# famoreno/stereo-vo

Measured on AMD Instinct MI355X. Metric: stereo pairs/sec @1280×960, higher is better.
Workload: dtype u8/f64

## Files before the change

### stereo_vo_amd/csrc/k_detect.hip

```cpp
#include <algorithm>
#include "svo_device.h"
#include "svo_kernels.h"
#include "../../include/svo_orb_tables.h"

__constant__ int c_umax[16];
__device__ __attribute__((aligned(16))) float4 g_brief_patf[SVO_BRIEF_NPAIRS];
__device__ __attribute__((aligned(16))) uint4 g_blur_gh[3 * 64], g_blur_gv[3 * 64];
#define SVO_DISC_E 256
__device__ uint32_t g_disc_m[SVO_DISC_E], g_disc_x[SVO_DISC_E];
#define DP_REACH SVO_BRIEF_REACH
#define DP_BW (2 * DP_REACH + 1)
#define DP_RW (DP_BW + 6)
#define DP_X0 (DP_REACH + 5)

hipError_t svo_upload_tables()
{
    hipError_t e = hipMemcpyToSymbol(HIP_SYMBOL(c_umax), svo_umax, sizeof(svo_umax));
    if (e != hipSuccess) return e;
    {
        static float4 pf[SVO_BRIEF_NPAIRS];
        for (int i = 0; i < SVO_BRIEF_NPAIRS; i++) pf[i] = make_float4((float)svo_brief_pat[i][0], (float)svo_brief_pat[i][2], (float)svo_brief_pat[i][1], (float)svo_brief_pat[i][3]);
        e = hipMemcpyToSymbol(HIP_SYMBOL(g_brief_patf), pf, sizeof(pf));
        if (e != hipSuccess) return e;
    }
// ... 322 lines not shown
{
    fast_reset(sm.score, sm.s_count, sm.s_nout);
    fast_stage<false>(sm.tile, src, pitch, gw, gh, x0, y0);
    asm volatile("s_waitcnt vmcnt(0)" ::: "memory");
    __syncthreads();
    fast_compute(c, sm.tile, sm.score, sm.list, sm.s_count, sm.s_nout, img, level, gw, gh, x0, y0, th_fast);
}

__device__ __forceinline__ void fast_compute(const DevCtx& c, uint8_t* tile, uint8_t* score, unsigned short* list, unsigned& s_count, unsigned& s_nout,
                                             int img, int level, int gw, int gh, int x0, int y0, int th_fast)
{
    uint32_t* out_keys = (uint32_t*)tile;
    const int tid = threadIdx.x;
    if (c.debug_mode == DBG_FAST_STOP_STAGED) return;
    const uint32_t th = (uint32_t)th_fast;
    const u16x2 t2h = { (unsigned short)(th << 8), (unsigned short)(th << 8) };
    const int gq = tid & (FT_NG - 1), rb = tid >> 4;
    const int e_base = rb * (FT_ROWS * FT_SP) + 4 * gq;
    uint32_t pe[FT_ROWS], po[FT_ROWS];
    {
        const uint32_t* col = (const uint32_t*)tile + rb * (FT_ROWS * (FT_LW / 4)) + gq;
        uint32_t cc[FT_ROWS + 6];
#pragma unroll
        for (int i = 0; i < FT_ROWS + 6; i++) cc[i] = col[i * (FT_LW / 4) + 1];
#pragma unroll
        for (int g = 0; g < FT_ROWS; g++) {
            const uint32_t Cp = col[(g + 3) * (FT_LW / 4)], C = cc[g + 3], Cn = col[(g + 3) * (FT_LW / 4) + 2], N = cc[g], S = cc[g + 6];
            const uint32_t Eo = __builtin_amdgcn_alignbyte(Cn, C, 3), Wo = __builtin_amdgcn_alignbyte(C, Cp, 1);
            const uint32_t Ee = __builtin_amdgcn_alignbyte(Cn, C, 2);
            pe[g] = quick_half(C << 8, N << 8, Ee, S << 8, Cp, t2h);
            po[g] = quick_half(C, N, Eo, S, Wo, t2h);
        }
    }
    auto entry_of = [&](int b) -> int { return e_base + ((b & 7) << 6) + (b >> 3); };
    uint32_t m_left = 0;
    {
        const uint32_t one2 = 0x00010001u;
        uint32_t me = 0, mo = 0;
#pragma unroll
        for (int g = FT_ROWS - 1; g >= 0; g--) {
            uint32_t fe, fo;
            asm("v_pk_min_u16 %0, %1, %2" : "=v"(fe) : "v"(pe[g]), "s"(one2));
            asm("v_pk_min_u16 %0, %1, %2" : "=v"(fo) : "v"(po[g]), "s"(one2));
            if (g == FT_ROWS - 1) { me = fe; mo = fo; }
            else {
                asm("v_lshl_or_b32 %0, %1, 1, %2" : "=v"(me) : "v"(me), "v"(fe));
                asm("v_lshl_or_b32 %0, %1, 1, %2" : "=v"(mo) : "v"(mo), "v"(fo));
            }
        }
        uint32_t m = me | (mo << 8);
        const int cnt = __popc(m), inc = wave_inclusive_scan(cnt);
        const int total = __builtin_amdgcn_readlane(inc, 63);
        if (total) {
            unsigned wbase = 0;
            if ((tid & 63) == 0) wbase = atomicAdd(&s_count, (unsigned)total);
            unsigned idx = (unsigned)__builtin_amdgcn_readfirstlane((int)wbase) + (unsigned)(inc - cnt);
            while (m && idx < FT_LIST_CAP) {
                const int b = __builtin_ctz(m); m &= m - 1;
                list[idx++] = (unsigned short)entry_of(b);
            }
            m_left = m;
        }
    }
    __syncthreads();
    const int ns_all = (int)s_count, ns = min(ns_all, FT_LIST_CAP);
    const bool overflow = ns_all > FT_LIST_CAP;
    if (c.debug_mode == DBG_FAST_STOP_COMPACTED) return;
    auto win_off = [&](int e) -> int { return (e >> 6) * FT_LW + (e & 63) + (3 * FT_LW + 4); };
    for (int i = tid; i < ns; i += FT_NT) {
        const int e = list[i];
        score[e] = (uint8_t)fast_score_lds(tile, win_off(e), th_fast);
    }
    if (__builtin_expect(overflow, 0)) {
        for (uint32_t m = m_left; m; m &= m - 1) {
            const int e = entry_of(__builtin_ctz(m));
            score[e] = (uint8_t)fast_score_lds(tile, win_off(e), th_fast);
        }
    }
    __syncthreads();
    if (c.debug_mode == DBG_FAST_STOP_SCORED) return;
    auto nms_round = [&](bool has, int e) {
        bool keep = false; uint32_t key = 0;
        if (has) {
            const int r = e >> 6, q = e & 63;
            const int nb = e - FT_SP - 1; int nbm = nb; asm volatile("" : "+v"(nbm));
            const int v = score[nbm + FT_SP + 1];
            const int n0 = score[nb], n1 = score[nbm + 1], n2 = score[nb + 2], n3 = score[nb + FT_SP], n4 = score[nb + FT_SP + 2];
            const int n5 = score[nb + 2 * FT_SP], n6 = score[nbm + 2 * FT_SP + 1], n7 = score[nb + 2 * FT_SP + 2];
            const int mx = max(max(max(n0, n1), max(n2, n3)), max(max(n4, n5), max(n6, n7)));
            const int x = x0 - 1 + q, y = y0 - 1 + r;
            keep = (v > mx) & (r >= 1) & (r <= FT_H) & (q >= 1) & (q <= FT_W) & (x < gw - SVO_EDGE) & (y < gh - SVO_EDGE);
            key = ((uint32_t)v << 24) | (0xFFFFFFu - (uint32_t)(y * gw + x));
        }
        const unsigned long long m = __ballot(keep);
        if (m) {
            unsigned b2 = 0;
            const int leader = __ffsll((long long)m) - 1;
            if ((tid & 63) == leader) b2 = atomicAdd(&s_nout, (unsigned)__popcll(m));
            b2 = __shfl(b2, leader, 64);
            if (keep) out_keys[b2 + __popcll(m & ((1ull << (tid & 63)) - 1ull))] = key;
        }
    };
    for (int base = 0; base < ns; base += FT_NT) {
        const int i = base + tid;
        nms_round(i < ns, i < ns ? (int)list[i] : 0);
    }
    if (__builtin_expect(overflow, 0)) {
        uint32_t m = m_left;
        while (__ballot(m != 0)) {
            const bool has = m != 0;
            const int e = has ? entry_of(__builtin_ctz(m)) : 0;
            m &= m - 1;
            nms_round(has, e);
        }
    }
    __syncthreads();
    if (tid < 64) {
        const unsigned nout = s_nout;
        if (nout != 0 && c.debug_mode != DBG_FAST_NO_PUBLISH) {
            const LevelGeom& g = c.lv[level];
            unsigned gbase = 0;
            if (tid == 0) gbase = atomicAdd(&c.cand_cnt[(img * SVO_MAX_LEVELS + level) * SVO_CNT_STRIDE], nout);
            gbase = __shfl(gbase, 0, 64);
            uint32_t* dst = c.cand_keys + (long long)img * c.cand_total + g.cand_off;
            for (unsigned i = tid; i < nout; i += 64) {
                if (gbase + i < (unsigned)g.cand_cap) dst[gbase + i] = out_keys[i];
                else raise_detect_status(c, img >> 1, SVO_ST_CAND_OVERFLOW);
            }
        }
    }
}

__global__ void __launch_bounds__(FT_NT) __attribute__((amdgpu_waves_per_eu(8, 8))) k_fast(DevCtx c)
{
    SVO_TL_SCOPE(c, TL_FAST, 0);
    __shared__ FastSmem sm;
    const uint32_t slot = blockIdx.x >> 3;
    const uint32_t work = c.debug_mode == DBG_LINEAR_TILES ? blockIdx.x : (((slot / FT_CHUNK) * 8 + (blockIdx.x & 7)) * FT_CHUNK + slot % FT_CHUNK);
    const int img = (int)fastdiv(work, c.div_tiles), tile_id = (int)work - img * c.n_tiles;
    if (img >= c.n_img || lane_idle(c, img >> 1)) return;
    const uint4 e = c.fast_tiles[tile_id];
    const uint4 tha = ((const uint4*)(c.fast_th_used + img * SVO_MAX_LEVELS))[0], thb = ((const uint4*)(c.fast_th_used + img * SVO_MAX_LEVELS))[1];
    const uint8_t* base0 = c.img0[img];
    const int level = (int)(e.z & 0xFFu);
    const uint32_t thv[8] = { tha.x, tha.y, tha.z, tha.w, thb.x, thb.y, thb.z, thb.w };
    uint32_t th = thv[0];
#pragma unroll
    for (int l = 1; l < SVO_MAX_LEVELS; l++) th = level == l ? thv[l] : th;
    const uint8_t* src = level == 0 ? base0 : c.pyr + (long long)img * c.pyr_bytes + e.w;
    const int pitch = level == 0 ? c.img0_pitch : (int)(e.z >> 8);
    fast_tile(c, sm, img, level, src, pitch, (int)(e.y & 0xFFFFu), (int)(e.y >> 16), (int)(e.x & 0xFFFFu), (int)(e.x >> 16), (int)th);
}

__global__ void __launch_bounds__(FT_NT) k_fast_redo(DevCtx c)
{
    SVO_TL_SCOPE(c, TL_FAST, 1);
    __shared__ FastSmem sm;
    const unsigned n = *c.redo_n;
    if (n == 0) return;
    int first = (int)blockIdx.x;
    for (unsigned e = 0; e < n; e++) {
        const uint32_t il = c.redo_list[e];
        const int img = (int)(il / SVO_MAX_LEVELS), level = (int)(il % SVO_MAX_LEVELS);
        const int nt = c.lv[level].tiles_x * c.lv[level].tiles_y;
        int t = first;
        int pitch; const uint8_t* src = level_ptr(c, img, level, pitch);
        const int tx = c.lv[level].tiles_x, gw = c.lv[level].w, gh = c.lv[level].h;
        for (; t < nt; t += (int)gridDim.x) {
            const int by = t / tx, bx = t - by * tx;
            fast_tile(c, sm, img, level, src, pitch, gw, gh, SVO_EDGE + bx * FT_W, SVO_EDGE + by * FT_H, c.fast_th);
            __syncthreads();
        }
        first = t - nt;
    }
}


__device__ __forceinline__ float harris_at(const uint8_t* img, int pitch, int x, int y)
{
    int a = 0, b = 0, cc = 0;
    for (int dy = -3; dy <= 3; dy++) {
        const uint8_t* pm = img + (long long)(y + dy - 1) * pitch + x, *p0 = pm + pitch, *pp = p0 + pitch;
#pragma unroll
        for (int dx = -3; dx <= 3; dx++) {
            const int Ix = ((int)p0[dx + 1] - (int)p0[dx - 1]) * 2 + ((int)pm[dx + 1] - (int)pm[dx - 1]) + ((int)pp[dx + 1] - (int)pp[dx - 1]);
            const int Iy = ((int)pp[dx] - (int)pm[dx]) * 2 + ((int)pp[dx - 1] - (int)pm[dx - 1]) + ((int)pp[dx + 1] - (int)pm[dx + 1]);
            a += Ix * Ix; b += Iy * Iy; cc += Ix * Iy;
        }
    }
    const float s = 1.0f / (4.0f * 7.0f * 255.0f);
    const float s4 = s * s * s * s;
    const float fa = (float)a, fb = (float)b, fc = (float)cc;
    const float tr = fa + fb;
    return (fa * fb - fc * fc - 0.04f * tr * tr) * s4;
}

__device__ __forceinline__ float harris_at_dw(const uint8_t* img, int pitch, int x, int y)
{
    const int xa = (x - 4) & ~3, o = (x - 4) & 3;
    int px[9][9];
#pragma unroll
    for (int r = 0; r < 9; r++) {
        const uint3 pw = *(const uint3*)(img + (long long)(y - 4 + r) * pitch + xa);
        const uint32_t w0 = pw.x, w1 = pw.y, w2 = pw.z;
        const uint32_t A = __builtin_amdgcn_alignbyte(w1, w0, o), B = __builtin_amdgcn_alignbyte(w2, w1, o), C = w2 >> (8 * o);
#pragma unroll
        for (int k = 0; k < 4; k++) { px[r][k] = (A >> (8 * k)) & 0xFF; px[r][4 + k] = (B >> (8 * k)) & 0xFF; }
        px[r][8] = C & 0xFF;
    }
    int a = 0, b = 0, cc = 0;
#pragma unroll
    for (int r = 1; r < 8; r++) {
#pragma unroll
        for (int q = 1; q < 8; q++) {
            const int Ix = (px[r][q + 1] - px[r][q - 1]) * 2 + (px[r - 1][q + 1] - px[r - 1][q - 1]) + (px[r + 1][q + 1] - px[r + 1][q - 1]);
            const int Iy = (px[r + 1][q] - px[r - 1][q]) * 2 + (px[r + 1][q - 1] - px[r - 1][q - 1]) + (px[r + 1][q + 1] - px[r - 1][q + 1]);
            a += __mul24(Ix, Ix); b += __mul24(Iy, Iy); cc += __mul24(Ix, Iy);
        }
    }
    const float s = 1.0f / (4.0f * 7.0f * 255.0f);
    const float s4 = s * s * s * s;
    const float fa = (float)a, fb = (float)b, fc = (float)cc;
    const float tr = fa + fb;
    return (fa * fb - fc * fc - 0.04f * tr * tr) * s4;
}

template <int SEL_MAX>
__device__ __forceinline__ int select_block(const DevCtx& c, int redo_pass, int img, int level, unsigned long long* keys, uint32_t* sel, unsigned* hist, int* scan_s, unsigned* sv)
{
    constexpr int SEL_TIE_MAX = 2 * SEL_MAX;
    unsigned& s_prefix = sv[0]; unsigned& s_need = sv[1]; unsigned& s_sel = sv[2]; unsigned& s_tie = sv[3]; unsigned& s_ntie = sv[4];
    const LevelGeom& g = c.lv[level];
    const int tid = threadIdx.x;
    const int il = img * SVO_MAX_LEVELS + level;
    if (redo_pass && !c.redo_flag[il]) return 0;
    unsigned nc = c.cand_cnt[il * SVO_CNT_STRIDE];
    if (nc > (unsigned)g.cand_cap) nc = g.cand_cap;
    const unsigned K = min(nc, (unsigned)(2 * g.quota));
    const uint32_t th_used = c.fast_th_used[il], th_base = (uint32_t)c.fast_th;
    if (!redo_pass && g.quota > 0 && th_used > th_base && nc < (unsigned)(2 * g.quota)) {
        if (tid == 0) {
            c.redo_flag[il] = 1; c.redo_list[atomicAdd(c.redo_n, 1u)] = (uint32_t)il;
            atomicAdd(c.redo_n + 1, 1u);
            c.cand_cnt[il * SVO_CNT_STRIDE] = 0; c.fast_th_used[il] = th_base; c.fast_th_dyn[il] = 0;
        }
        return 0;
    }
    if (K == 0 || g.quota <= 0) { if (tid == 0) { c.lvl_n[il] = 0; c.sel_n[il] = 0; c.fast_th_dyn[il] = 0; } return 0; }
    const uint32_t* ck = c.cand_keys + (long long)img * c.cand_total + g.cand_off;
    uint32_t* tie = (uint32_t*)keys;
    for (int i = tid; i < 256; i += blockDim.x) hist[i] = 0;
    if (tid == 0) { s_sel = 0; s_tie = 0; }
    __syncthreads();
    for (unsigned base = tid; base < nc; base += 8 * 512) {
        uint32_t k[8];
#pragma unroll
        for (int u = 0; u < 8; u++) { const unsigned i = base + u * 512; k[u] = i < nc ? ck[i] : 0u; }
#pragma unroll
        for (int u = 0; u < 8; u++) if (base + u * 512 < nc) atomicAdd(&hist[k[u] >> 24], 1u);
    }
    __syncthreads();
    if (c.debug_mode == DBG_SELECT_STOP_HIST) return 0;
    unsigned prefix = 0, mask = 0, need = K;
    {
        const int mine = tid < 256 ? (int)hist[255 - tid] : 0;
        int tot;
        const int before = block_exclusive_scan(mine, scan_s, &tot);
        if (tid < 256 && (unsigned)before < need && need <= (unsigned)(before + mine)) { s_prefix = (unsigned)(255 - tid) << 24; s_need = need - (unsigned)before; s_ntie = (unsigned)mine; }
        const unsigned M = 3u * (unsigned)g.quota + 32u;
        if (tid < 256 && (unsigned)before < M && M <= (unsigned)(before + mine)) c.fast_th_dyn[il] = (uint32_t)(255 - tid) > th_base ? (uint32_t)(255 - tid) : 0u;
        if (tid == 0 && (unsigned)tot < M) {
            const unsigned dens = max(hist[min(th_used, 255u)], 1u), lower = (M - (unsigned)tot) / dens + 1u;
            c.fast_th_dyn[il] = th_used > th_base + lower ? th_used - lower : 0u;
        }
        __syncthreads();
        prefix = s_prefix; need = s_need; mask = 0xFF000000u;
    }
    const unsigned n_tie = s_ntie;
    uint32_t cutoff;
    const unsigned K_ties = (K - need) + n_tie;
    if (K_ties <= (unsigned)SEL_MAX) {
        cutoff = prefix;
        for (unsigned base = tid; base < nc; base += 8 * 512) {
            uint32_t k[8];
#pragma unroll
            for (int u = 0; u < 8; u++) { const unsigned i = base + u * 512; k[u] = i < nc ? ck[i] : 0u; }
#pragma unroll
            for (int u = 0; u < 8; u++) if (base + u * 512 < nc && k[u] >= cutoff) sel[atomicAdd(&s_sel, 1u)] = k[u];
        }
        __syncthreads();
        return (int)K_ties;
    }
    if (tid == 0) raise_detect_status(c, img >> 1, SVO_ST_CAND_OVERFLOW);
    if (n_tie <= SEL_TIE_MAX) {
        for (unsigned base = tid; base < nc; base += 8 * 512) {
            uint32_t k[8];
#pragma unroll
            for (int u = 0; u < 8; u++) { const unsigned i = base + u * 512; k[u] = i < nc ? ck[i] : 0u; }
#pragma unroll
            for (int u = 0; u < 8; u++) {
                if (base + u * 512 >= nc) continue;
                if ((k[u] & 0xFF000000u) > prefix) sel[atomicAdd(&s_sel, 1u)] = k[u];
                else if ((k[u] & 0xFF000000u) == prefix) tie[atomicAdd(&s_tie, 1u)] = k[u];
            }
        }
        __syncthreads();
        for (int shift = 16; shift >= 0; shift -= 8) {
            for (int i = tid; i < 256; i += blockDim.x) hist[i] = 0;
            __syncthreads();
            for (unsigned i = tid; i < n_tie; i += blockDim.x) { const uint32_t k = tie[i]; if ((k & mask) == prefix) atomicAdd(&hist[(k >> shift) & 255u], 1u); }
            __syncthreads();
            const int mine = tid < 256 ? (int)hist[255 - tid] : 0;
            int tot;
            const int before = block_exclusive_scan(mine, scan_s, &tot);
            if (tid < 256 && (unsigned)before < need && need <= (unsigned)(before + mine)) { s_prefix = prefix | ((unsigned)(255 - tid) << shift); s_need = need - (unsigned)before; }
            __syncthreads();
            prefix = s_prefix; need = s_need; mask |= 255u << shift;
            __syncthreads();
        }
        cutoff = prefix;
        for (unsigned i = tid; i < n_tie; i += blockDim.x) { const uint32_t k = tie[i]; if (k >= cutoff) sel[atomicAdd(&s_sel, 1u)] = k; }
        __syncthreads();
    } else {
        for (int shift = 16; shift >= 0; shift -= 8) {
            for (int i = tid; i < 256; i += blockDim.x) hist[i] = 0;
            __syncthreads();
            for (unsigned i = tid; i < nc; i += blockDim.x) { const uint32_t k = ck[i]; if ((k & mask) == prefix) atomicAdd(&hist[(k >> shift) & 255u], 1u); }
            __syncthreads();
            const int mine = tid < 256 ? (int)hist[255 - tid] : 0;
            int tot;
            const int before = block_exclusive_scan(mine, scan_s, &tot);
            if (tid < 256 && (unsigned)before < need && need <= (unsigned)(before + mine)) { s_prefix = prefix | ((unsigned)(255 - tid) << shift); s_need = need - (unsigned)before; }
            __syncthreads();
            prefix = s_prefix; need = s_need; mask |= 255u << shift;
            __syncthreads();
        }
        cutoff = prefix;
        for (unsigned i = tid; i < nc; i += blockDim.x) { const uint32_t k = ck[i]; if (k >= cutoff) { const unsigned sl = atomicAdd(&s_sel, 1u); if (sl < SEL_MAX) sel[sl] = k; } }
        __syncthreads();
    }
    return (int)K;
}

template <int SEL_MAX>
__global__ void __launch_bounds__(512) k_select(DevCtx c, int redo_pass)
{
    SVO_TL_SCOPE(c, TL_SELECT, redo_pass);
    __shared__ unsigned long long keys[SEL_MAX];
    __shared__ uint32_t sel[SEL_MAX];
    __shared__ unsigned hist[256];
    __shared__ int scan_s[32];
    __shared__ unsigned sv[5];
    const int level = blockIdx.y, img = blockIdx.x, tid = threadIdx.x;
    if (lane_idle(c, img >> 1)) return;
    const int K = select_block<SEL_MAX>(c, redo_pass, img, level, keys, sel, hist, scan_s, sv);
    if (K <= 0) return;
    uint32_t* gsel = c.sel_keys + ((long long)img * SVO_MAX_LEVELS + level) * c.sel_max;
    for (int i = tid; i < K; i += blockDim.x) gsel[i] = sel[i];
    if (tid == 0) c.sel_n[img * SVO_MAX_LEVELS + level] = K;
}

__global__ void __launch_bounds__(256) k_harris(DevCtx c)
{
    SVO_TL_SCOPE(c, TL_HARRIS, 0);
    const int img = blockIdx.x, level = blockIdx.z, i = blockIdx.y * 256 + threadIdx.x;
    if (lane_idle(c, img >> 1)) return;
    const LevelGeom& g = c.lv[level];
    const int K = g.quota > 0 ? c.sel_n[img * SVO_MAX_LEVELS + level] : 0;
    if ((int)(blockIdx.y * 256) >= K) return;
    if (i >= K) return;
    const long long o = ((long long)img * SVO_MAX_LEVELS + level) * c.sel_max + i;
    const uint32_t pos = 0xFFFFFFu - (c.sel_keys[o] & 0xFFFFFFu);
    const int x = (int)(pos % (uint32_t)g.w), y = (int)(pos / (uint32_t)g.w);
    int pitch; const uint8_t* lim = level_ptr(c, img, level, pitch);
    const bool aligned = (((uintptr_t)lim | (uintptr_t)pitch) & 3) == 0;
    const float r = aligned ? harris_at_dw(lim, pitch, x, y) : harris_at(lim, pitch, x, y);
    c.sel_resp[o] = ((unsigned long long)ord32(r) << 32) | (unsigned long long)(0xFFFFFFFFu - pos);
}

#define SS_NB 1024
template <int SEL_MAX>
__device__ __forceinline__ void rank_block(const DevCtx& c, int img, int level, int K, const unsigned long long (&mykey)[SEL_MAX / 512],
                                           unsigned long long* keys, unsigned long long* tmp, int* cnt, int* off, int* scan_s, unsigned* sv)
{
    unsigned& s_mn = sv[0]; unsigned& s_mx = sv[1]; unsigned& s_mnp = sv[2]; int& s_np = *(int*)(sv + 3);
    const int tid = threadIdx.x;
    const LevelGeom& g = c.lv[level];
    if (tid == 0) { s_mn = 0xFFFFFFFFu; s_mx = 0u; s_mnp = 0xFFFFFFFFu; s_np = 0; }
    for (int i = tid; i < SS_NB; i += blockDim.x) cnt[i] = 0;
    __syncthreads();
    int mypos[SEL_MAX / 512], myb[SEL_MAX / 512];
    unsigned lmn = 0xFFFFFFFFu, lmx = 0u, lmnp = 0xFFFFFFFFu; int lnp = 0;
#pragma unroll
    for (int it = 0; it < SEL_MAX / 512; it++) {
        const int i = tid + it * 512;
        if (i < K) {
            const unsigned h = (unsigned)(mykey[it] >> 32);
            lmn = min(lmn, h); lmx = max(lmx, h);
            if (h >= 0x80000000u) { lmnp = min(lmnp, h); lnp++; }
        }
    }
#pragma unroll
    for (int o = 32; o > 0; o >>= 1) {
        lmn = min(lmn, (unsigned)__shfl_xor((int)lmn, o, 64)); lmx = max(lmx, (unsigned)__shfl_xor((int)lmx, o, 64));
        lmnp = min(lmnp, (unsigned)__shfl_xor((int)lmnp, o, 64)); lnp += __shfl_xor(lnp, o, 64);
    }
    if (c.debug_mode == DBG_SSORT_STOP_RANGE) return;
    if ((tid & 63) == 0) { atomicMin(&s_mn, lmn); atomicMax(&s_mx, lmx); atomicMin(&s_mnp, lmnp); atomicAdd(&s_np, lnp); }
    __syncthreads();
    const unsigned mn = s_np >= g.quota ? s_mnp : s_mn;
    const float scale = (float)(SS_NB - 1) / ((float)(s_mx - mn) + 1.0f);
#pragma unroll
    for (int it = 0; it < SEL_MAX / 512; it++) {
        const int i = tid + it * 512;
        if (i < K) {
            const unsigned h = (unsigned)(mykey[it] >> 32);
            const int b = h < mn ? SS_NB - 1 : SS_NB - 1 - min((int)((float)(h - mn) * scale), SS_NB - 1);
            myb[it] = b; mypos[it] = atomicAdd(&cnt[b], 1);
        }
    }
    __syncthreads();
    if (c.debug_mode == DBG_SSORT_STOP_BUCKETS) return;
    int run = 0;
    for (int base = 0; base < SS_NB; base += 512) {
        int tot;
        const int o = block_exclusive_scan(cnt[base + tid], scan_s, &tot);
        off[base + tid] = run + o;
        run += tot;
        __syncthreads();
    }
    if (c.debug_mode == DBG_SSORT_STOP_OFFSETS) return;
#pragma unroll
    for (int it = 0; it < SEL_MAX / 512; it++) { const int i = tid + it * 512; if (i < K) tmp[off[myb[it]] + mypos[it]] = mykey[it]; }
    __syncthreads();
    if (c.debug_mode == DBG_SSORT_STOP_SCATTER) return;
#pragma unroll
    for (int it = 0; it < SEL_MAX / 512; it++) {
        const int i = tid + it * 512;
        if (i < K) {
            const int b0 = off[myb[it]], nb = cnt[myb[it]];
            if (b0 >= min(K, g.quota)) continue;
            int greater = 0;
            for (int q = 0; q < nb; q++) greater += tmp[b0 + q] > mykey[it] ? 1 : 0;
            keys[b0 + greater] = mykey[it];
        }
    }
    __syncthreads();
    if (c.debug_mode == DBG_SSORT_STOP_RANK) return;
    const int nout = min(K, g.quota);
    for (int i = tid; i < nout; i += blockDim.x) {
        const unsigned long long k = keys[i];
        const uint32_t pos = 0xFFFFFFFFu - (uint32_t)(k & 0xFFFFFFFFull);
        c.lvl_pos[(long long)img * c.raw_cap + g.slot_off + i] = (pos % (uint32_t)g.w) | ((pos / (uint32_t)g.w) << 16);
        c.lvl_resp[(long long)img * c.raw_cap + g.slot_off + i] = inv_ord32((uint32_t)(k >> 32));
    }
    if (tid == 0) c.lvl_n[img * SVO_MAX_LEVELS + level] = nout;
}


#define LDS_FN __host__ __device__ constexpr int
#define LDS_CU_BYTES (160 * 1024)
template <int SEL_MAX>
struct LdsSelectSort {
    LDS_FN n_keys() const { return SEL_MAX; }
    LDS_FN n_tmp() const { return SEL_MAX; }
    LDS_FN total() const { return 8 * (n_keys() + n_tmp()); }
};
static_assert(LdsSelectSort<2048>{}.total() == 32768 && LdsSelectSort<4096>{}.total() == 65536 && LdsSelectSort<8192>{}.total() == 131072, "k_select_sort LDS totals");
static_assert(LdsSelectSort<8192>{}.total() + 8336 <= LDS_CU_BYTES, "gfx950: 160 KB of LDS per CU");

template <int SEL_MAX>
__global__ void __launch_bounds__(512) k_select_sort(DevCtx c)
{
    SVO_TL_SCOPE(c, TL_SELECT_SORT, 0);
    extern __shared__ __attribute__((aligned(16))) unsigned char ss_smem[];
    constexpr LdsSelectSort<SEL_MAX> L{};
    unsigned long long* keys = (unsigned long long*)ss_smem, *tmp = keys + L.n_keys();
    __shared__ int cnt[SS_NB], off[SS_NB], scan_s[32];
    __shared__ unsigned sv[4];
    const int level = blockIdx.y, img = blockIdx.x, tid = threadIdx.x;
    if (c.lv[level].quota <= 0 || lane_idle(c, img >> 1)) return;
    const int K = c.sel_n[img * SVO_MAX_LEVELS + level];
    if (K <= 0) return;
    const unsigned long long* gk = c.sel_resp + ((long long)img * SVO_MAX_LEVELS + level) * c.sel_max;
    unsigned long long mykey[SEL_MAX / 512];
#pragma unroll
    for (int it = 0; it < SEL_MAX / 512; it++) { const int i = tid + it * 512; mykey[it] = i < K ? gk[i] : 0ull; }
    rank_block<SEL_MAX>(c, img, level, K, mykey, keys, tmp, cnt, off, scan_s, sv);
}


#define DP_PW 12
#define DP_LROWS 48
typedef int dp_v4i __attribute__((ext_vector_type(4)));

__device__ __forceinline__ float atan2_deg(float y, float x)
{
    const float p1 = 57.283627f, p3 = -18.667446f, p5 = 8.9140005f, p7 = -2.5397246f;
    const float ax = fabsf(x), ay = fabsf(y);
    const bool steep = !(ax >= ay);
    const float cq = (steep ? ax : ay) / ((steep ? ay : ax) + 2.220446e-16f);
    const float c2 = cq * cq;
    float a = (((p7 * c2 + p5) * c2 + p3) * c2 + p1) * cq;
    if (steep) a = 90.0f - a;
    if (x < 0.0f) a = 180.0f - a;
    if (y < 0.0f) a = 360.0f - a;
    return a;
}

__device__ __forceinline__ void sincos_f32(float x, float& sn, float& cs)
{
    const int k = (int)(x * 0.63661977f + 0.5f);
    const float fk = (float)k;
    const float r = ((x - fk * 1.5703125f) - fk * 4.837512969970703125e-4f) - fk * 7.54978995489188216e-8f;
    const float z = r * r;
    const float sp = ((-1.9515295891e-4f * z + 8.3321608736e-3f) * z - 1.6666654611e-1f) * z * r + r;
    const float cp = ((2.443315711809948e-5f * z - 1.388731625493765e-3f) * z + 4.166664568298827e-2f) * z * z - 0.5f * z + 1.0f;
    const bool odd = k & 1;
    const float s0 = odd ? cp : sp, c0 = odd ? sp : cp;
    sn = (k & 2) ? -s0 : s0;
    cs = (((k + 1) & 2) != 0) ? -c0 : c0;
}

__device__ __forceinline__ uint32_t udot4(uint32_t a, uint32_t b, uint32_t acc)
{
    return __builtin_amdgcn_udot4(a, b, acc, false);
}

template <int NW, bool TL>
__global__ void __launch_bounds__(NW * 64) k_describe(DevCtx c, FastDiv gx_div, int pre, int kpw)
{
    SVO_TL_SCOPE(c, TL_DESCRIBE, pre);
    __shared__ __attribute__((aligned(16))) uint32_t raw32[NW][2][DP_LROWS * DP_PW + 4];
    __shared__ __attribute__((aligned(16))) float4 s_pat[SVO_BRIEF_NPAIRS];
    __shared__ uint32_t s_disc_m[SVO_DISC_E], s_disc_x[SVO_DISC_E];
    static_assert(NW * 64 == SVO_BRIEF_NPAIRS && NW * 64 == SVO_DISC_E, "one table entry per thread");
    __shared__ __attribute__((aligned(16))) uint4 s_gh[TL ? 3 * 64 : 1], s_gv[TL ? 3 * 64 : 1];
    if (c.idle.w[0] | c.idle.w[1]) {
        const int img_b = c.debug_mode == DBG_LINEAR_TILES ? (int)(blockIdx.x / gx_div.d) : (int)(fastdiv(blockIdx.x >> 3, gx_div) * 8 + (blockIdx.x & 7));
        if (img_b < c.n_img && lane_idle(c, img_b >> 1)) return;
    }
    s_pat[threadIdx.x] = g_brief_patf[threadIdx.x]; s_disc_m[threadIdx.x] = g_disc_m[threadIdx.x]; s_disc_x[threadIdx.x] = g_disc_x[threadIdx.x];
    if (TL && threadIdx.x < 3 * 64) { s_gh[threadIdx.x] = g_blur_gh[threadIdx.x]; s_gv[threadIdx.x] = g_blur_gv[threadIdx.x]; }
    __syncthreads();
    const int wid = __builtin_amdgcn_readfirstlane((int)(threadIdx.x >> 6)), lane = threadIdx.x & 63;
    int img, bx;
    if (c.debug_mode == DBG_LINEAR_TILES) { img = blockIdx.x / gx_div.d; bx = blockIdx.x - img * gx_div.d; }
    else { const uint32_t r = blockIdx.x >> 3, grp = fastdiv(r, gx_div); bx = (int)(r - grp * gx_div.d); img = (int)(grp * 8 + (blockIdx.x & 7)); }
    if (img >= c.n_img) return;
    const int lane_id = img >> 1, vl0 = lane_id * c.oct_cap;
    const int n_end = __builtin_amdgcn_readfirstlane(pre ? c.desc_n[img] : c.n_slots);
    const int slot0 = (bx * NW + wid) * kpw;
    if (slot0 >= n_end) return;
    const int slot1 = min(slot0 + kpw, n_end);
    const long long fo0 = pre ? feat_base(c, vl0, 1 - c.lane[lane_id].prev_slot, img & 1) : 0;
    dp_v4i GH[3], GV[3];
#pragma unroll
    for (int t = 0; t < 3; t++) { if (!TL) { GH[t] = *(const dp_v4i*)&g_blur_gh[t * 64 + lane]; GV[t] = *(const dp_v4i*)&g_blur_gv[t * 64 + lane]; } else { GH[t] = dp_v4i{0, 0, 0, 0}; GV[t] = GH[t]; } }
#pragma unroll
    for (int t = 0; t < 3; t++) if (!TL) asm volatile("" : "+v"(GH[t]), "+v"(GV[t]));
    uint32_t w_pos = 0, w_lvl = 0;
    if (slot0 + lane < slot1) {
        if (pre) { const uint2 w = c.desc_work[(long long)img * c.raw_cap + slot0 + lane]; w_pos = w.x; w_lvl = w.y; }
        else w_pos = c.lvl_pos[(long long)img * c.raw_cap + slot0 + lane];
    }
    asm volatile("" : "+v"(w_pos), "+v"(w_lvl));
    auto item = [&](int slot, int& live, int& x, int& y, int& level) {
        const uint32_t pos = (uint32_t)__builtin_amdgcn_readlane((int)w_pos, slot - slot0);
        int lv = 0, ok = 1;
        if (pre) lv = __builtin_amdgcn_readlane((int)w_lvl, slot - slot0);
        else {
#pragma unroll
            for (int l = 1; l < SVO_MAX_LEVELS; l++) if (l < c.n_levels && slot >= c.lv[l].slot_off) lv = l;
            lv = __builtin_amdgcn_readfirstlane(lv);
            ok = __builtin_amdgcn_readfirstlane(slot - c.lv[lv].slot_off < c.lvl_n[img * SVO_MAX_LEVELS + lv] ? 1 : 0);
        }
        level = lv; live = ok; x = (int)(pos & 0xFFFFu); y = (int)(pos >> 16);
    };
    const uint8_t* base0; const uint8_t* pyr0 = c.pyr + (long long)img * c.pyr_bytes;
    {
        const uint64_t b = (uint64_t)(uintptr_t)c.img0[img];
        base0 = (const uint8_t*)(uintptr_t)(((uint64_t)(uint32_t)__builtin_amdgcn_readfirstlane((int)(b >> 32)) << 32) | (uint32_t)__builtin_amdgcn_readfirstlane((int)(uint32_t)b));
    }
    const int cr0 = (lane * 171) >> 9, cq0 = lane - 3 * cr0, cr1 = ((lane + 64) * 171) >> 9, cq1 = lane + 64 - 3 * cr1;
    auto stage = [&](uint32_t* dst, int x, int y, int level) {
        const int pitch = level == 0 ? c.img0_pitch : c.lv[level].pitch;
        const uint8_t* lim = level == 0 ? base0 : pyr0 + c.lv[level].offset;
        const uint8_t* org = lim + (uint32_t)((y - (DP_REACH + 3)) * pitch + (x - DP_X0));
        const uint32_t lb = (uint32_t)__builtin_amdgcn_readfirstlane((int)(uint32_t)(uintptr_t)(__attribute__((address_space(3))) uint32_t*)dst);
        glds16_asm(org + (uint32_t)(cr0 * pitch + 16 * cq0), lb);
        glds16_asm(org + (uint32_t)(cr1 * pitch + 16 * cq1), lb + 1024);
        if (lane < DP_RW * 3 - 128) glds16_asm(org + (uint32_t)(42 * pitch + 32), lb + 2048);
    };
    static_assert(DP_RW * 3 - 128 == 1, "the third DMA instruction carries chunk 128 alone");
    int live, x, y, level;
    item(slot0, live, x, y, level);
    if (live) stage(raw32[wid][0], x, y, level);
    const int n16 = lane & 15, q4 = lane >> 4;
    for (int slot = slot0; slot < slot1; slot++) {
        uint32_t* R32 = raw32[wid][(slot - slot0) & 1];
        int live_n = 0, x_n = 0, y_n = 0, level_n = 0;
        if (slot + 1 < slot1) item(slot + 1, live_n, x_n, y_n, level_n);
        live_n = __builtin_amdgcn_readfirstlane(live_n); x_n = __builtin_amdgcn_readfirstlane(x_n); y_n = __builtin_amdgcn_readfirstlane(y_n); level_n = __builtin_amdgcn_readfirstlane(level_n);
        asm volatile("s_waitcnt vmcnt(0)" ::: "memory");
        wave_lds_sync();
        if (live_n) stage(raw32[wid][(slot - slot0 + 1) & 1], x_n, y_n, level_n);
        if (live) {
            uint32_t m10u = 0; int m01 = 0, msum = 0;
#pragma unroll
            for (int i = 0; i < 4; i++) {
                const int en = i * 64 + lane;
                const int vr = en >> 3, d = en & 7;
                const uint32_t px = R32[(vr + 6) * DP_PW + 2 + d];
                const uint32_t s = udot4(px, s_disc_m[en], 0u);
                m10u = udot4(px, s_disc_x[en], m10u);
                msum += (int)s;
                m01 += __mul24(vr - 15, (int)s);
            }
            const int m10 = wave_sum_uniform((int)m10u - 15 * msum);
            m01 = wave_sum_uniform(m01);
            float angle, sn, cs;
            if (c.debug_mode == DBG_DESCRIBE_NO_TRIG) { angle = (float)(m10 & 255); sn = (float)(m01 & 255) * 0.001f; cs = 1.f - sn; }
            else { angle = atan2_deg((float)m01, (float)m10); sincos_f32(angle * 0.017453292f, sn, cs); }
            dp_v4i S[3][3];
            {
                if (TL) {
#pragma unroll
                    for (int t = 0; t < 3; t++) GH[t] = *(const dp_v4i*)&s_gh[t * 64 + lane];
                }
                const dp_v4i seed = { 128, 128, 128, 128 };
#pragma unroll
                for (int mt = 0; mt < 3; mt++) {
                    dp_v4i X = *(const dp_v4i*)&R32[(16 * mt + n16) * DP_PW + 4 * q4];
                    X ^= (int)0x80808080;
#pragma unroll
                    for (int nt = 0; nt < 3; nt++) S[mt][nt] = __builtin_amdgcn_mfma_i32_16x16x64_i8(X, GH[nt], seed, 0, 0, 0);
                }
            }
            wave_lds_sync();
            uint8_t* Bl = (uint8_t*)R32;
// ... 774 lines not shown
void launch_fastorb_anms(const DevCtx& c, uint32_t* scratch3, hipStream_t st)
{
    const LdsFastorbAnms L{c.max_kps};
    const size_t one = L.scratch_array_words(c.n_img, c.cand_total);
    hipLaunchKernelGGL(k_fastorb_anms, dim3(c.n_levels, c.n_img), dim3(1024), (size_t)L.total(), st, c, scratch3, scratch3 + one, scratch3 + 2 * one, L.n_keys());
}
size_t fastorb_anms_scratch_words(int n_img, int cand_total) { return LdsFastorbAnms::scratch_words(n_img, cand_total); }

#define FK_W SVO_FK_W
#define FK_H SVO_FK_H
#define FK_NT 256
#define FK_HALO_MAX 16
#define FK_LW (FK_W + 2 * FK_HALO_MAX)
#define FK_LH (FK_H + 2 * FK_HALO_MAX)
static_assert(FK_LW % 4 == 0 && FK_LW <= 128 && FK_W == 64 && FK_NT == 256 && FK_W * FK_H <= 65536, "k_faster's thread mapping: 32 threads x 4 bytes per window row, one thread per column and four rows per pass, 16-bit list entries");

__device__ __forceinline__ bool faster_run12(uint32_t m)
{
    const uint32_t mm = m | (m << 16);
    const uint32_t x2 = mm & (mm >> 1), x4 = x2 & (x2 >> 2), x8 = x4 & (x4 >> 4), x12 = x8 & (x4 >> 8);
    return (x12 & 0xFFFFu) != 0u;
}
#define FKO(dx, dy) ((dy) * FK_LW + (dx))
__device__ __forceinline__ bool faster_is_corner(const uint8_t* p, int th)
{
    const int c0 = p[0], hi = c0 + th, lo = c0 - th;
    const int pn = p[FKO(0, -3)], pe = p[FKO(3, 0)], ps = p[FKO(0, 3)], pw = p[FKO(-3, 0)];
    const int nb = (pn > hi) + (pe > hi) + (ps > hi) + (pw > hi), nd = (pn < lo) + (pe < lo) + (ps < lo) + (pw < lo);
    if (nb < 3 && nd < 3) return false;
    constexpr int off[16] = { FKO(0, -3), FKO(1, -3), FKO(2, -2), FKO(3, -1), FKO(3, 0), FKO(3, 1), FKO(2, 2), FKO(1, 3),
                              FKO(0, 3), FKO(-1, 3), FKO(-2, 2), FKO(-3, 1), FKO(-3, 0), FKO(-3, -1), FKO(-2, -2), FKO(-1, -3) };
    uint32_t b = 0, d = 0;
#pragma unroll
    for (int i = 0; i < 16; i++) { const int v = p[off[i]]; b |= (uint32_t)(v > hi) << i; d |= (uint32_t)(v < lo) << i; }
    return faster_run12(b) || faster_run12(d);
}
#undef FKO

__device__ __forceinline__ float faster_klt_response(const uint8_t* p, int win)
{
    int gxx = 0, gxy = 0, gyy = 0;
    for (int v = -win; v <= win; v++) {
        const uint8_t* r = p + v * FK_LW;
        int left = r[-win - 1], mid = r[-win];
        for (int u = -win; u <= win; u++) {
            const int right = r[u + 1];
            const int dx = right - left, dy = (int)r[u + FK_LW] - (int)r[u - FK_LW];
            gxx += dx * dx; gxy += dx * dy; gyy += dy * dy;
            left = mid; mid = right;
        }
    }
    const int side = 2 * win + 1;
    const float K = 0.5f / (float)(side * side);
    const float Gxx = (float)gxx * K, Gxy = (float)gxy * K, Gyy = (float)gyy * K;
    const float t = Gxx + Gyy;
    const float de = Gxx * Gyy - Gxy * Gxy;
    const float rad = t * t - 4.0f * de;
    return 0.5f * (t - sqrtf(rad < 0.0f ? 0.0f : rad));
}

__global__ void __launch_bounds__(FK_NT) k_faster(DevCtx c, unsigned long long* cand64, int th, int win)
{
    SVO_TL_SCOPE(c, TL_FAST, 2);
    __shared__ __attribute__((aligned(16))) uint8_t tile[FK_LH * FK_LW];
    __shared__ unsigned short list[FK_W * FK_H];
    __shared__ unsigned s_n, s_base;
    const int tid = threadIdx.x;
    const int img = (int)fastdiv(blockIdx.x, c.div_tiles), tile_id = (int)blockIdx.x - img * c.n_tiles;
    if (img >= c.n_img || lane_idle(c, img >> 1)) return;
    const uint4 e = c.fast_tiles[tile_id];
    const int level = (int)(e.z & 0xFFu), gw = (int)(e.y & 0xFFFFu), gh = (int)(e.y >> 16), x0 = (int)(e.x & 0xFFFFu), y0 = (int)(e.x >> 16);
    const uint8_t* src = level == 0 ? c.img0[img] : c.pyr + (long long)img * c.pyr_bytes + e.w;
    const int pitch = level == 0 ? c.img0_pitch : (int)(e.z >> 8);
    const int halo = max(3, win + 1), lw = FK_W + 2 * halo, lh = FK_H + 2 * halo;
    if (tid == 0) s_n = 0;
    {
        const int q4 = (tid & 31) * 4, gx = x0 - halo + q4;
        if (q4 < lw)
            for (int r = tid >> 5; r < lh; r += FK_NT / 32) {
                const int gy = y0 - halo + r;
                uint32_t v = 0;
                if (gy >= 0 && gy < gh) {
                    const uint8_t* row = src + (size_t)gy * (size_t)pitch;
#pragma unroll
                    for (int k = 0; k < 4; k++) if (gx + k >= 0 && gx + k < gw) v |= (uint32_t)row[gx + k] << (8 * k);
                }
                *(uint32_t*)(tile + r * FK_LW + q4) = v;
            }
    }
    __syncthreads();
    const int lx = tid & 63, x = x0 + lx;
#pragma unroll 2
    for (int k = 0; k < FK_H / 4; k++) {
        const int ly = (tid >> 6) + 4 * k, y = y0 + ly;
        const bool is = x < gw - 3 && y < gh - 3 && faster_is_corner(tile + (ly + halo) * FK_LW + lx + halo, th);
        const unsigned slot = wave_append_slot(is, &s_n);
        if (is) list[slot] = (unsigned short)(ly * FK_W + lx);
    }
    __syncthreads();
    const unsigned n = s_n;
    if (n == 0) return;
    const LevelGeom& g = c.lv[level];
    if (tid == 0) s_base = atomicAdd(&c.cand_cnt[(img * SVO_MAX_LEVELS + level) * SVO_CNT_STRIDE], n);
    __syncthreads();
    const unsigned gbase = s_base;
    unsigned long long* dst = cand64 + (long long)img * c.cand_total + g.cand_off;
    for (unsigned i = tid; i < n; i += FK_NT) {
        const int ent = list[i], cy = ent / FK_W, cx = ent % FK_W, px = x0 + cx, py = y0 + cy;
        float resp = 0.0f;
        if (px >= win + 1 && py >= win + 1 && px < gw - win - 1 && py < gh - win - 1) resp = faster_klt_response(tile + (cy + halo) * FK_LW + cx + halo, win);
        if (gbase + i < (unsigned)g.cand_cap) dst[gbase + i] = ((unsigned long long)ord32(resp) << 32) | (unsigned long long)(0xFFFFFFFFu - (uint32_t)(py * gw + px));
        else raise_detect_status(c, img >> 1, SVO_ST_CAND_OVERFLOW);
    }
}

void launch_begin_frame(const DevCtx& c, const uint8_t* const* ptrs, unsigned flags, const LaneMask& drop_prev, hipStream_t st)
{
    ImgPtrs ip;
    for (int i = 0; i < 2 * SVO_MAX_LANES; i++) ip.p[i] = (ptrs && i < c.n_img) ? ptrs[i] : nullptr;
    const int n = c.n_img * SVO_MAX_LEVELS;
    int blocks = (n + 255) / 256;
    if (flags & (SVO_RUN_MATCH | SVO_RUN_TRACK)) {
        const size_t n16 = (size_t)c.n_lanes * c.oct_cap * 3 * c.max_kps / 4;
        blocks = std::max(blocks, (int)std::min<size_t>((n16 + 1023) / 1024, 2048));
    }
    hipLaunchKernelGGL(k_begin_frame, dim3(blocks), dim3(256), 0, st, c, ip, flags, drop_prev);
}

void launch_resize(const DevCtx& c, int level, hipStream_t st)
{
    const LevelGeom& d = c.lv[level];
    const int ntx = (d.w + RZ_W - 1) / RZ_W, per_img = ntx * ((d.h + RZ_H - 1) / RZ_H);
    const long long total = (long long)per_img * c.n_img, unit = 8 * RZ_CHUNK;
    hipLaunchKernelGGL(k_resize, dim3((unsigned)((total + unit - 1) / unit * unit)), dim3(256), 0, st, c, level, make_fastdiv((uint32_t)per_img), make_fastdiv((uint32_t)ntx));
}

void launch_fast(const DevCtx& c, hipStream_t st)
{
    if (c.n_tiles <= 0) return;
    const long long total = (long long)c.n_tiles * c.n_img, unit = 8 * FT_CHUNK;
    hipLaunchKernelGGL(k_fast, dim3((unsigned)((total + unit - 1) / unit * unit)), dim3(FT_NT), 0, st, c);
}

template <class F> static auto select_form(int sel_max, F f)
{
    if (sel_max > 4096) return f(std::integral_constant<int, 8192>());
    if (sel_max > 2048) return f(std::integral_constant<int, 4096>());
    return f(std::integral_constant<int, 2048>());
}

void launch_select(const DevCtx& c, hipStream_t st)
{
    const dim3 grid(c.n_img, c.n_levels);
    auto select = [&](int pass) { select_form(c.sel_max, [&](auto s) { hipLaunchKernelGGL(k_select<decltype(s)::value>, grid, dim3(512), 0, st, c, pass); }); };
    select(0);
    hipLaunchKernelGGL(k_fast_redo, dim3(4096), dim3(FT_NT), 0, st, c);
    select(1);
    hipLaunchKernelGGL(k_harris, dim3(c.n_img, c.sel_max / 256, c.n_levels), dim3(256), 0, st, c);
    select_form(c.sel_max, [&](auto s) { constexpr int S = decltype(s)::value; hipLaunchKernelGGL(k_select_sort<S>, grid, dim3(512), (size_t)LdsSelectSort<S>{}.total(), st, c); });
}

void launch_describe(const DevCtx& c, const Knobs& k, int pre, hipStream_t st)
{
    if (c.n_slots <= 0) return;
    const int kpw = k.desc_kpw, per = 4 * kpw, gx = (c.n_slots + per - 1) / per, img8 = (c.n_img + 7) / 8 * 8;
    if (k.desc_tl) hipLaunchKernelGGL((k_describe<4, true>), dim3((unsigned)((long long)gx * img8)), dim3(256), 0, st, c, make_fastdiv((uint32_t)gx), (pre && !c.fast_orb) ? 1 : 0, kpw);
    else hipLaunchKernelGGL((k_describe<4, false>), dim3((unsigned)((long long)gx * img8)), dim3(256), 0, st, c, make_fastdiv((uint32_t)gx), (pre && !c.fast_orb) ? 1 : 0, kpw);
}

void launch_sad_patch(const DevCtx& c, hipStream_t st)
{
    const int n = c.fast_orb ? c.max_kps : std::min(c.n_slots, c.max_kps);
    if (n <= 0) return;
    hipLaunchKernelGGL(k_sad_patch, dim3((n + 31) / 32, c.n_lanes * c.oct_cap * 2), dim3(256), 0, st, c);
}

void launch_publish_img0(const DevCtx& c, const uint8_t* const* ptrs, hipStream_t st)
{
    ImgPtrs ip;
    for (int i = 0; i < 2 * SVO_MAX_LANES; i++) ip.p[i] = i < c.n_img ? ptrs[i] : nullptr;
    hipLaunchKernelGGL(k_publish_img0, dim3((c.n_img + 255) / 256), dim3(256), 0, st, c, ip);
}
void launch_sad_patch_slot(const DevCtx& c, int which, hipStream_t st)
{
    hipLaunchKernelGGL(k_sad_patch_slot, dim3((c.max_kps + 31) / 32, c.n_lanes * c.oct_cap * 2), dim3(256), 0, st, c, which);
}

template <class T> static LdsChunkedNms<typename T::Key> chunked_nms_layout(const DevCtx& c) { return {FO_PMAX, c.max_kps}; }
static int nms_pmax(const DevCtx& c)
{
    int n = 64;
    if (c.fast_orb) { for (int l = 0; l < c.n_levels; l++) if (c.lv[l].quota > n) n = c.lv[l].quota; } else n = c.n_slots;
    int p = 64; while (p < n) p <<= 1; return p;
}
template <class F> static auto nms_rowsort_form(int pmax, F f)
{
    if (pmax > 8192) return f(std::integral_constant<int, 16>());
    if (pmax > 4096) return f(std::integral_constant<int, 8>());
    return f(std::integral_constant<int, 4>());
}

int nms_rowsort_items(const DevCtx& c) { return nms_rowsort_form(nms_pmax(c), [](auto n) { return (int)decltype(n)::value; }); }

size_t nms_rowsort_scratch_bytes(int n_img, int oct_cap, int n_keys) { return LdsNmsRowsort{n_keys}.scratch_bytes((size_t)n_img * oct_cap); }

hipError_t configure_nms_rowsort(const DevCtx& c)
{
    hipError_t e = svo_raise_dyn_smem((const void*)k_fastorb_nms, chunked_nms_layout<FastOrbKeys>(c).total());
    if (e != hipSuccess) return e;
    e = svo_raise_dyn_smem((const void*)k_fastorb_anms, LdsFastorbAnms{c.max_kps}.total());
    if (e != hipSuccess) return e;
    e = select_form(c.sel_max, [](auto s) { constexpr int S = decltype(s)::value; return svo_raise_dyn_smem((const void*)k_select_sort<S>, LdsSelectSort<S>{}.total()); });
    if (e != hipSuccess) return e;
    const int pmax = nms_pmax(c);
    if (pmax > 16384) return hipErrorInvalidValue;
    return nms_rowsort_form(pmax, [&](auto n) { return svo_raise_dyn_smem((const void*)k_nms_rowsort<decltype(n)::value>, LdsNmsRowsort{pmax}.total()); });
}

void launch_nms_rowsort(const DevCtx& c, const Knobs& k, int do_nms, int min_distance, int pre, hipStream_t st)
{
    const LdsNmsRowsort L{nms_pmax(c)};
    const int pmax = L.ns_max;
    const int nt = (pmax <= 2048 && k.nms_nt == 512) ? 512 : 1024;
    const int mode = c.fast_orb ? (do_nms == 3 ? 3 : 0) : do_nms, pre_pass = (pre && !c.fast_orb) ? 1 : 0;
    nms_rowsort_form(pmax, [&](auto n) {
        hipLaunchKernelGGL(k_nms_rowsort<decltype(n)::value>, dim3(c.n_img, c.n_oct), dim3(nt), (size_t)L.total(), st, c, mode, min_distance, pmax, pre_pass, L.wide_in_scratch() ? c.big_scratch : (uint8_t*)nullptr);
    });
}

void launch_half(const DevCtx& c, int level, hipStream_t st)
{
    const LevelGeom& d = c.lv[level];
    hipLaunchKernelGGL(k_half, dim3(((d.w + 3) / 4 + 255) / 256, d.h, c.n_img), dim3(256), 0, st, c, level);
}

void launch_fastorb_nms(const DevCtx& c, int do_nms, int min_distance, hipStream_t st)
{
    const auto L = chunked_nms_layout<FastOrbKeys>(c);
    hipLaunchKernelGGL(k_fastorb_nms, dim3(c.n_levels, c.n_img), dim3(1024), (size_t)L.total(), st, c, min_distance, do_nms, L.ns_max, L.acc_max);
}

void launch_faster(const DevCtx& c, unsigned long long* cand64, int fast_th, int klt_win, hipStream_t st)
{
    if (c.n_tiles <= 0) return;
    hipLaunchKernelGGL(k_faster, dim3((unsigned)((long long)c.n_tiles * c.n_img)), dim3(FK_NT), 0, st, c, cand64, fast_th, klt_win);
}

hipError_t configure_faster_nms(const DevCtx& c) { return svo_raise_dyn_smem((const void*)k_faster_nms, chunked_nms_layout<FasterKeys>(c).total()); }

void launch_faster_nms(const DevCtx& c, const unsigned long long* cand64, int do_nms, int min_distance, hipStream_t st)
{
    const auto L = chunked_nms_layout<FasterKeys>(c);
    hipLaunchKernelGGL(k_faster_nms, dim3(c.n_levels, c.n_img), dim3(1024), (size_t)L.total(), st, c, cand64, min_distance, do_nms, L.ns_max, L.acc_max);
}
```

Before: 74500.

## Fold FAST redo into Harris kernel and redo-select into select_sort

The separate FAST-redo kernel and second select pass are removed. Redo tiles are now processed by extra blocks of the Harris kernel, and the redo level's selection plus Harris scoring is done inside the select_sort kernel. The goal is to cut the select pipeline from five launches to three and run the redo work concurrently with normal Harris scoring. In exchange, select_sort does serial select plus Harris work for redo levels, and the Harris kernel carries FastSmem LDS that can lower its occupancy.

New measurement: 74470. No clear change (-0.0%).

```diff
diff --git a/stereo_vo_amd/csrc/k_detect.hip b/stereo_vo_amd/csrc/k_detect.hip
--- a/stereo_vo_amd/csrc/k_detect.hip
+++ b/stereo_vo_amd/csrc/k_detect.hip
@@ -498,13 +498,11 @@
     fast_tile(c, sm, img, level, src, pitch, (int)(e.y & 0xFFFFu), (int)(e.y >> 16), (int)(e.x & 0xFFFFu), (int)(e.x >> 16), (int)th);
 }
 
-__global__ void __launch_bounds__(FT_NT) k_fast_redo(DevCtx c)
-{
-    SVO_TL_SCOPE(c, TL_FAST, 1);
-    __shared__ FastSmem sm;
+__device__ __forceinline__ void fast_redo_worker(const DevCtx& c, FastSmem& sm, int worker, int n_workers)
+{
     const unsigned n = *c.redo_n;
     if (n == 0) return;
-    int first = (int)blockIdx.x;
+    int first = worker;
     for (unsigned e = 0; e < n; e++) {
         const uint32_t il = c.redo_list[e];
         const int img = (int)(il / SVO_MAX_LEVELS), level = (int)(il % SVO_MAX_LEVELS);
@@ -512,7 +510,7 @@
         int t = first;
         int pitch; const uint8_t* src = level_ptr(c, img, level, pitch);
         const int tx = c.lv[level].tiles_x, gw = c.lv[level].w, gh = c.lv[level].h;
-        for (; t < nt; t += (int)gridDim.x) {
+        for (; t < nt; t += n_workers) {
             const int by = t / tx, bx = t - by * tx;
             fast_tile(c, sm, img, level, src, pitch, gw, gh, SVO_EDGE + bx * FT_W, SVO_EDGE + by * FT_H, c.fast_th);
             __syncthreads();
@@ -589,6 +587,7 @@
             c.redo_flag[il] = 1; c.redo_list[atomicAdd(c.redo_n, 1u)] = (uint32_t)il;
             atomicAdd(c.redo_n + 1, 1u);
             c.cand_cnt[il * SVO_CNT_STRIDE] = 0; c.fast_th_used[il] = th_base; c.fast_th_dyn[il] = 0;
+            c.sel_n[il] = 0;
         }
         return 0;
     }
@@ -689,9 +688,9 @@
 }
 
 template <int SEL_MAX>
-__global__ void __launch_bounds__(512) k_select(DevCtx c, int redo_pass)
-{
-    SVO_TL_SCOPE(c, TL_SELECT, redo_pass);
+__global__ void __launch_bounds__(512) k_select(DevCtx c)
+{
+    SVO_TL_SCOPE(c, TL_SELECT, 0);
     __shared__ unsigned long long keys[SEL_MAX];
     __shared__ uint32_t sel[SEL_MAX];
     __shared__ unsigned hist[256];
@@ -699,20 +698,24 @@
     __shared__ unsigned sv[5];
     const int level = blockIdx.y, img = blockIdx.x, tid = threadIdx.x;
     if (lane_idle(c, img >> 1)) return;
-    const int K = select_block<SEL_MAX>(c, redo_pass, img, level, keys, sel, hist, scan_s, sv);
+    const int K = select_block<SEL_MAX>(c, 0, img, level, keys, sel, hist, scan_s, sv);
     if (K <= 0) return;
     uint32_t* gsel = c.sel_keys + ((long long)img * SVO_MAX_LEVELS + level) * c.sel_max;
     for (int i = tid; i < K; i += blockDim.x) gsel[i] = sel[i];
     if (tid == 0) c.sel_n[img * SVO_MAX_LEVELS + level] = K;
 }
 
-__global__ void __launch_bounds__(256) k_harris(DevCtx c)
-{
-    SVO_TL_SCOPE(c, TL_HARRIS, 0);
+#define FAST_REDO_WORKERS 4096
+__host__ __device__ __forceinline__ int fast_redo_workers(const DevCtx& c) { const long long t = (long long)c.n_tiles * c.n_img; return (int)(t < FAST_REDO_WORKERS ? t : FAST_REDO_WORKERS); }
+
+__device__ __forceinline__ void harris_block(const DevCtx& c)
+{
     const int img = blockIdx.x, level = blockIdx.z, i = blockIdx.y * 256 + threadIdx.x;
     if (lane_idle(c, img >> 1)) return;
     const LevelGeom& g = c.lv[level];
-    const int K = g.quota > 0 ? c.sel_n[img * SVO_MAX_LEVELS + level] : 0;
+    const uint32_t redo = c.redo_flag[img * SVO_MAX_LEVELS + level];
+    const int n = c.sel_n[img * SVO_MAX_LEVELS + level];
+    const int K = (g.quota > 0 && !redo) ? n : 0;
     if ((int)(blockIdx.y * 256) >= K) return;
     if (i >= K) return;
     const long long o = ((long long)img * SVO_MAX_LEVELS + level) * c.sel_max + i;
@@ -722,6 +725,18 @@
     const bool aligned = (((uintptr_t)lim | (uintptr_t)pitch) & 3) == 0;
     const float r = aligned ? harris_at_dw(lim, pitch, x, y) : harris_at(lim, pitch, x, y);
     c.sel_resp[o] = ((unsigned long long)ord32(r) << 32) | (unsigned long long)(0xFFFFFFFFu - pos);
+}
+
+__global__ void __launch_bounds__(256) k_harris(DevCtx c)
+{
+    SVO_TL_SCOPE(c, TL_HARRIS, 0);
+    __shared__ FastSmem sm;
+    const int hy = c.sel_max / 256;
+    const int nw = fast_redo_workers(c), w = (int)((blockIdx.y * gridDim.z + blockIdx.z) * gridDim.x + blockIdx.x);
+    const unsigned n_redo = w < nw ? *c.redo_n : 0u;
+    if ((int)blockIdx.y < hy) harris_block(c);
+    if (n_redo == 0 || threadIdx.x >= FT_NT) return;
+    fast_redo_worker(c, sm, w, nw);
 }
 
 #define SS_NB 1024
@@ -826,12 +841,35 @@
     __shared__ unsigned sv[4];
     const int level = blockIdx.y, img = blockIdx.x, tid = threadIdx.x;
     if (c.lv[level].quota <= 0 || lane_idle(c, img >> 1)) return;
-    const int K = c.sel_n[img * SVO_MAX_LEVELS + level];
-    if (K <= 0) return;
-    const unsigned long long* gk = c.sel_resp + ((long long)img * SVO_MAX_LEVELS + level) * c.sel_max;
+    const int il = img * SVO_MAX_LEVELS + level;
+    const long long o = (long long)il * c.sel_max;
     unsigned long long mykey[SEL_MAX / 512];
-#pragma unroll
-    for (int it = 0; it < SEL_MAX / 512; it++) { const int i = tid + it * 512; mykey[it] = i < K ? gk[i] : 0ull; }
+    const uint32_t redo = c.redo_flag[il];
+    int K = c.sel_n[il];
+    if (redo) {
+        static_assert(256 <= SS_NB && 5 <= SS_NB && 4 * SEL_MAX <= 8 * L.n_tmp(), "select_block's arrays fit the ranking's");
+        uint32_t* sel = (uint32_t*)tmp;
+        K = select_block<SEL_MAX>(c, 1, img, level, keys, sel, (unsigned*)cnt, scan_s, (unsigned*)off);
+        if (K <= 0) return;
+        const LevelGeom& g = c.lv[level];
+        int pitch; const uint8_t* lim = level_ptr(c, img, level, pitch);
+#pragma unroll 1
+        for (int i = tid; i < K; i += 512) {
+            const uint32_t k32 = sel[i], pos = 0xFFFFFFu - (k32 & 0xFFFFFFu);
+            const float r = harris_at(lim, pitch, (int)(pos % (uint32_t)g.w), (int)(pos / (uint32_t)g.w));
+            const unsigned long long k64 = ((unsigned long long)ord32(r) << 32) | (unsigned long long)(0xFFFFFFFFu - pos);
+            keys[i] = k64; c.sel_keys[o + i] = k32; c.sel_resp[o + i] = k64;
+        }
+        if (tid == 0) c.sel_n[il] = K;
+#pragma unroll
+        for (int it = 0; it < SEL_MAX / 512; it++) { const int i = tid + it * 512; mykey[it] = i < K ? keys[i] : 0ull; }
+        __syncthreads();
+    } else {
+        if (K <= 0) return;
+        const unsigned long long* gk = c.sel_resp + o;
+#pragma unroll
+        for (int it = 0; it < SEL_MAX / 512; it++) { const int i = tid + it * 512; mykey[it] = i < K ? gk[i] : 0ull; }
+    }
     rank_block<SEL_MAX>(c, img, level, K, mykey, keys, tmp, cnt, off, scan_s, sv);
 }
 
@@ -1912,11 +1950,9 @@
 void launch_select(const DevCtx& c, hipStream_t st)
 {
     const dim3 grid(c.n_img, c.n_levels);
-    auto select = [&](int pass) { select_form(c.sel_max, [&](auto s) { hipLaunchKernelGGL(k_select<decltype(s)::value>, grid, dim3(512), 0, st, c, pass); }); };
-    select(0);
-    hipLaunchKernelGGL(k_fast_redo, dim3(4096), dim3(FT_NT), 0, st, c);
-    select(1);
-    hipLaunchKernelGGL(k_harris, dim3(c.n_img, c.sel_max / 256, c.n_levels), dim3(256), 0, st, c);
+    select_form(c.sel_max, [&](auto s) { hipLaunchKernelGGL(k_select<decltype(s)::value>, grid, dim3(512), 0, st, c); });
+    const int per_plane = c.n_img * c.n_levels, redo_planes = per_plane > 0 ? (fast_redo_workers(c) + per_plane - 1) / per_plane : 0;
+    hipLaunchKernelGGL(k_harris, dim3(c.n_img, std::max(c.sel_max / 256, redo_planes), c.n_levels), dim3(256), 0, st, c);
     select_form(c.sel_max, [&](auto s) { constexpr int S = decltype(s)::value; hipLaunchKernelGGL(k_select_sort<S>, grid, dim3(512), (size_t)LdsSelectSort<S>{}.total(), st, c); });
 }
 
```
